# rpng/open_vins

Hardware: AMD Instinct MI355X
Metric: MSCKF features/sec per EKF update (30-clone state) (higher is better)
Workload: dtype f64; 1 GPU; BASELINE.json configs[2]: 2-camera radtan rig, 30-clone window, 2000 MSCKF features/update, N=248, D=208, online cam extrinsic+intrinsic calib + IMU intrinsics in the state, FEJ; features_total=2000, features_this_rank=2000, clones=30, cameras=2, state_dim=248, measurements_total=100362, parallelism=single GPU

## Files before the change

open_vins_amd/csrc/api_context.inc:

```
using namespace ovg;

static thread_local std::string g_err = "";
static int set_err(int code, const std::string &msg) {
  g_err = msg;
  return code;
}

#define HIPCHK(expr)                                                                                         \
  do {                                                                                                       \
    hipError_t _e = (expr);                                                                                  \
    if (_e != hipSuccess) {                                                                                  \
      return set_err(OVGPU_ERR_HIP, std::string(#expr) + " -> " + hipGetErrorString(_e) + " (" __FILE__ ":" + \
                                        std::to_string(__LINE__) + ")");                                     \
    }                                                                                                        \
  } while (0)

namespace {

template <class T>
struct PinBuf {
  T *p = nullptr;
  size_t cap = 0;
  hipError_t reserve(size_t n) {
    if (n <= cap) return hipSuccess;
// ... 186 lines not shown
  int tree_G2 = 0;
  hipStream_t stream2 = nullptr;
  hipEvent_t ev_rows = nullptr;
  bool gram_il = true;
  bool gram_blocks_only = false;
  bool fuse_chol_inputs = true;
  hipEvent_t ev_fork = nullptr, ev_join = nullptr;
  DevBuf<int32_t> leaf_flags;
  int tree_overlap = -1;
  bool tree_nodes_overlap = false, tree_nodes2_overlap = false;
  DevBuf<int32_t> tree_flags;
  DevBuf<int32_t> tree_err;
  int tree_G = 0;
  bool tree_pipelined = true;
  int compress_gram = 1;
  DevBuf<double> gram_part, gram_G, gram_rho, Yaug2, Lw;
  double prior_pivot_tol = 1e-13;
  int last_route = OVGPU_COMPRESS_GRAM;
  bool whiten = true;
  bool gram_is_whitened = false;
  bool prior_on_side = false;
  int feat_variant = 0;
  int feat_nt_max = 0;
  bool featy_ok = false;
  int featy_skip = 0;
  int featy_grid = 0;
  size_t featy_lds = 0;
  DevBuf<double> fs_tq;
  DevBuf<int32_t> fs_inst;
  DevBuf<double> featyb_ws;
  int featy_big = 0;
  bool no_feat_kernel = false;
  bool raw_enable = true;
  int raw_work_const = 12;
  bool raw_veto = false;
  bool raw_one_region = false;
  bool raw_cols_ok = false;
  bool raw_tables_ok = false;
  int raw_j0 = 0;
  int raw_ncls = 0, raw_ntc[RAW_MAXCLS + 1] = {0}, raw_ld[RAW_MAXCLS + 1] = {0}, raw_rcol[RAW_MAXCLS + 1] = {0};
  int64_t raw_base[RAW_MAXCLS + 1] = {0}, raw_rows[RAW_MAXCLS + 1] = {0};
  std::vector<uint8_t> h_cls_of_clone;
  DevBuf<uint8_t> cls_of_clone;
  DevBuf<int32_t> raw_featbase, raw_dst;
  DevBuf<double> Hraw;
  DevBuf<gram::GramRegionWG> gram_wg;
  int gram_wg_n = 0, gram_wg_tiles = 0;
  gram::GramRegionSum raw_rs;
  bool last_stack_raw = false;
  DevBuf<int32_t> feat_counter, fs_minfo, fs_meas_feat, fs_pos;
  DevBuf<int32_t> fs_slots;
  std::vector<int32_t> h_order;
  std::vector<uint16_t> h_cc;
  DevBuf<double> fs_rows, fs_V, fs_z, fs_w;
  void *comm = nullptr;
  struct LoopComm *loop = nullptr;
  int comm_rank = 0, comm_world = 1;
  DevBuf<double> comm_buf;
  DevBuf<int32_t> chol_prog;
  DevBuf<int32_t> ctrl;
  unsigned ctrl_clean = 0;
  unsigned ctrl_pre = 0;
  DevBuf<double> chol_uinv;
  DevBuf<double> chol_wide_A, chol_wide_Y;
  bool chol_wide = true;
  int64_t chol_wide_count = 0;
// ... 305 lines not shown
```

open_vins_amd/csrc/api_debug.inc:

```
int ovgpu_debug_option(ovgpu_ctx *c, const char *name, int64_t value, int64_t *old_value) {
  if (!c || !name) return set_err(OVGPU_ERR_INVALID, "null argument");
  const std::string n(name);
  if (n == "chol_follow_spin_limit") {
    if (old_value) *old_value = c->chol_spin_limit;
    if (value >= 0) c->chol_spin_limit = (int)std::min<int64_t>(value, 1 << 30);
  } else if (n == "slam_chunked_fail_chunk") {
    if (old_value) *old_value = c->chunk_fail_inject;
    c->chunk_fail_inject = value >= 0 ? (int)std::min<int64_t>(value, 1 << 20) : -1;
  } else if (n == "slam_chunked_fallbacks") {
    if (old_value) *old_value = c->chunk_fallbacks;
    if (value >= 0) c->chunk_fallbacks = value;
  } else if (n == "delayed_init_fused") {
    if (old_value) *old_value = c->init_fused_on ? 1 : 0;
    if (value >= 0) c->init_fused_on = value != 0;
  } else if (n == "delayed_init_fused_steps") {
    if (old_value) *old_value = c->init_fused_steps;
    if (value >= 0) c->init_fused_steps = value;
  } else if (n == "delayed_init_chain_steps") {
    if (old_value) *old_value = c->init_chain_steps;
    if (value >= 0) c->init_chain_steps = value;
  } else if (n == "gram_interleaved") {
    if (old_value) *old_value = c->gram_il ? 1 : 0;
    if (value >= 0) c->gram_il = value != 0;
  } else if (n == "layout_fpw") {
// ... 12 lines not shown
    if (old_value) *old_value = c->raw_enable ? 1 : 0;
    if (value >= 0) c->raw_enable = value != 0, c->raw_one_region = value == 2;
  } else if (n == "anchored_fast") {
    if (old_value) *old_value = c->anchored_fast ? 1 : 0;
    if (value >= 0) c->anchored_fast = value != 0;
  } else if (n == "gram_blocks_only") {
    if (old_value) *old_value = c->gram_blocks_only ? 1 : 0;
    if (value >= 0) c->gram_blocks_only = value != 0;
  } else if (n == "stage_timing_period") {
    if (old_value) *old_value = c->timing_period;
    if (value >= 1) c->timing_period = (int)value, c->timing_seq = 0;
  } else if (n == "fuse_chol_inputs") {
    if (old_value) *old_value = c->fuse_chol_inputs ? 1 : 0;
    if (value >= 0) c->fuse_chol_inputs = value != 0;
  } else if (n == "featy_big") {
    if (old_value) *old_value = c->featy_big;
    if (value >= 0) c->featy_big = (int)value;
  } else if (n == "upload_kernel") {
    if (old_value) *old_value = c->up_kernel;
    if (value >= 0) c->up_kernel = value != 0;
  } else if (n == "layout_every_update") {
    if (old_value) *old_value = c->layout_every_update;
    if (value >= 0) c->layout_every_update = value != 0;
  } else if (n == "tri_waves") {
    if (old_value) *old_value = c->tri_waves;
    if (value >= 0 && value <= 16) c->tri_waves = (int)value;
  } else if (n == "featy_skip") {
#ifdef OVG_FEAT_ABLATE
    if (old_value) *old_value = c->featy_skip;
    if (value >= 0) c->featy_skip = (int)value;
#else
    return set_err(OVGPU_ERR_INVALID, "featy_skip: ablation switches exist in a developer build only (-DOVG_FEAT_ABLATE)");
#endif
  } else if (n == "raw_work_const") {
    if (old_value) *old_value = c->raw_work_const;
    if (value >= 0) c->raw_work_const = (int)value;
  } else if (n == "last_stack_raw") {
    if (old_value) *old_value = c->last_stack_raw ? 1 : 0;
  } else if (n == "raw_gram_tile_rows") {
    int64_t t = 0;
    if (c->raw_tables_ok)
      for (int k = 0; k <= RAW_NEG; k++) t += c->raw_rows[k] * (int64_t)(c->raw_ntc[k] * (c->raw_ntc[k] + 1) / 2);
    if (old_value) *old_value = t;
  } else if (n == "stack_is_f32") {
    if (old_value) *old_value = c->stack_is_f32 ? 1 : 0;
  } else if (n == "last_feature_kernel") {
    if (old_value) *old_value = c->last_feat_kernel;
  } else if (n == "chol_wide") {
    if (old_value) *old_value = c->chol_wide ? 1 : 0;
    if (value >= 0) c->chol_wide = value != 0;
  } else if (n == "chol_wide_factorisations") {
    if (old_value) *old_value = c->chol_wide_count;
    if (value >= 0) c->chol_wide_count = value;
  } else if (n == "tsqr_leaves") {
    if (old_value) *old_value = c->tsqr_last_W;
  } else if (n == "tsqr_rows_per_node") {
    if (old_value) *old_value = c->tsqr_last_rpn;
  } else if (n == "tsqr_last_leaf_kernel") {
    if (old_value) *old_value = c->tsqr_last_leaf;
  } else if (n == "tsqr_last_tree") {
    if (old_value) *old_value = c->tsqr_last_tree;
  } else if (n == "tsqr_last_qh") {
    if (old_value) *old_value = c->tsqr_last_qh;
  } else if (n == "chol_timeouts") {
    if (old_value) *old_value = c->chol_timeouts;
  } else {
    return set_err(OVGPU_ERR_INVALID, "unknown debug option");
  }
  return OVGPU_OK;
}

int ovgpu_debug_cycles(ovgpu_ctx *c, int enable, long long *out512) {
  if (!c) return set_err(OVGPU_ERR_INVALID, "null ctx");
  HIPCHK(hipSetDevice(c->device));
  HIPCHK(upload_sync(c, c->stream));
  if (out512 && c->dbg_cycles.p) HIPCHK(hipMemcpy(out512, c->dbg_cycles.p, 512 * sizeof(long long), hipMemcpyDeviceToHost));
  if (enable) {
    HIPCHK(c->dbg_cycles.reserve(512));
    HIPCHK(hipMemset(c->dbg_cycles.p, 0, 512 * sizeof(long long)));
  } else if (!out512) {
    c->dbg_cycles.release();
  }
  return OVGPU_OK;
}

__global__ void k_clock_probe(long long *out, int iters) {
  const long long c0 = clock64(), w0 = wall_clock64();
  unsigned x = threadIdx.x + 1;
  for (int i = 0; i < iters; i++) x = x * 1664525u + 1013904223u;
  const long long c1 = clock64(), w1 = wall_clock64();
  if (threadIdx.x == 0) out[0] = c1 - c0, out[1] = w1 - w0, out[2] = (long long)x;
}
__global__ void __launch_bounds__(256) k_clock_probe_load(long long *out, int iters) {
  typedef double d4 __attribute__((ext_vector_type(4)));
  d4 a0 = {0, 0, 0, 0}, a1 = a0, a2 = a0, a3 = a0;
  const double x = 1.0 + 1e-9 * threadIdx.x, y = 1.0 - 1e-9 * threadIdx.x;
  const long long c0 = clock64(), w0 = wall_clock64();
  for (int i = 0; i < iters; i++) {
    a0 = __builtin_amdgcn_mfma_f64_16x16x4f64(x, y, a0, 0, 0, 0);
    a1 = __builtin_amdgcn_mfma_f64_16x16x4f64(y, x, a1, 0, 0, 0);
    a2 = __builtin_amdgcn_mfma_f64_16x16x4f64(x, x, a2, 0, 0, 0);
    a3 = __builtin_amdgcn_mfma_f64_16x16x4f64(y, y, a3, 0, 0, 0);
  }
  const long long c1 = clock64(), w1 = wall_clock64();
  if (blockIdx.x == 0 && threadIdx.x == 0) out[0] = c1 - c0, out[1] = w1 - w0;
  if (a0[0] + a1[1] + a2[2] + a3[3] == 12345.678) out[2] = 1;
}
__global__ void k_probe_empty(int *sink) {
  if (sink == nullptr && threadIdx.x == 12345) *sink = 0;
}
__global__ void k_chase_init(int32_t *buf, int n, int stride, int step) {
  const int i = blockIdx.x * blockDim.x + threadIdx.x;
  if (i < n) buf[(size_t)i * stride] = (int32_t)(((long long)i + step) % n);
}
__global__ void k_chase(const int32_t *buf, int stride, int hops, long long *out) {
  if (threadIdx.x != 0) return;
  int i = 0;
  for (int h = 0; h < 64; h++) i = __builtin_nontemporal_load(buf + (size_t)i * stride);
// ... 111 lines not shown
```

open_vins_amd/csrc/api_pipeline.inc:

```
static int enqueue_triangulate(ovgpu_ctx *c, const double *seed_pA = nullptr, const int32_t *seed_anchor = nullptr) {
  if (c->F == 0) return OVGPU_OK;
  TriParams p;
  p.seed_pA = seed_pA, p.seed_anchor = seed_anchor, p.anchor_pre = c->anchor_pre.p;
  p.F = c->F, p.C = c->C, p.K = c->K;
  p.meas_offsets = c->meas_offsets.p, p.meas_cc = c->meas_cc.p, p.uvn = c->uvn.p, p.tab_cc = c->tab_cc.p;
  p.p_FinA = c->pA.p, p.p_FinG = c->pG.p, p.anchor_meas = c->anchor.p, p.status = c->status.p;
  p.opt = c->dopt;
  const size_t lds = (size_t)c->K * c->C * 12 * sizeof(double);
  int wpb = c->tri_waves;
  if (wpb == 0) {
    wpb = 4;
    const int room = c->num_cu - 6;
    for (int w = 4; w <= 8 && room > 0; w *= 2) {
      const int blocks = (c->F + w - 1) / w;
      if (blocks <= room) {
        if (4 * blocks >= 3 * room) wpb = w;
        break;
      }
    }
  }
  hipLaunchKernelGGL(k_triangulate, dim3((c->F + wpb - 1) / wpb), dim3(64 * wpb), lds, c->stream, p);
  HIPCHK(hipGetLastError());
  return OVGPU_OK;
}
// ... 230 lines not shown
  HIPCHK(c->gram_part.reserve((size_t)G * NP * 256));
  HIPCHK(c->gram_G.reserve((size_t)LG * LG));
  if (c->stack_is_f32) {
    const int LDF = c->stack_ldf, NTM = LDF / 32, P = gram32::gram32_parts(NTM), slots = P * gram32::G32_NW * gram32::G32_MAXT;
    if (c->gram32_ntm != NTM || c->gram32_P != P) {
      std::vector<int32_t> tab((size_t)slots);
      gram32::gram32_tile_table(NTM, P, tab.data());
      HIPCHK(c->gram32_tiles.reserve((size_t)slots));
      HIPCHK(hipMemcpyAsync(c->gram32_tiles.p, tab.data(), sizeof(int32_t) * slots, hipMemcpyHostToDevice, c->stream));
      HIPCHK(upload_sync(c, c->stream));
      c->gram32_ntm = NTM, c->gram32_P = P;
    }
    const int64_t by_rows = (c->rows_total + gram32::G32_ROWS_WG - 1) / gram32::G32_ROWS_WG;
    const int64_t by_cus = std::min<int64_t>((2 * c->num_cu + P - 1) / P, (c->rows_total + 127) / 128);
    const int Gw = (int)std::max<int64_t>(1, std::max(by_rows, by_cus));
    HIPCHK(c->gram32_part.reserve((size_t)P * Gw * gram32::G32_NW * gram32::G32_MAXT * 1024));
    static bool attr32 = false;
    if (!attr32) {
      (void)hipFuncSetAttribute((const void *)gram32::k_gram_f32, hipFuncAttributeMaxDynamicSharedMemorySize, 160 * 1024);
      attr32 = true;
    }
    gram32::Gram32Params q;
    q.H = c->Hbig32.p, q.part = c->gram32_part.p, q.tiles = c->gram32_tiles.p, q.rows_total = c->rows_total, q.LDF = LDF, q.LD = LD;
    hipLaunchKernelGGL(gram32::k_gram_f32, dim3(Gw, P), dim3(gram32::G32_NTH), gram32::gram32_lds_bytes(LDF), c->stream, q);
    hipLaunchKernelGGL(gram32::k_gram_f32_reduce, dim3(slots, 4), dim3(256), 0, c->stream, (const int32_t *)c->gram32_tiles.p, Gw,
                       (const float *)c->gram32_part.p, c->gram_G.p, LG);
    HIPCHK(hipGetLastError());
    return factor ? set_err(OVGPU_ERR_CAPACITY, "the fp32 Gram variant feeds the on-device update only") : OVGPU_OK;
  }
  if (c->last_stack_raw) {
    HIPCHK(c->gram_part.reserve((size_t)std::max(c->gram_wg_tiles, 1) * 256));
    static bool attr_r = false;
    if (!attr_r) {
      (void)hipFuncSetAttribute((const void *)gram::k_gram_regions, hipFuncAttributeMaxDynamicSharedMemorySize, 160 * 1024);
      attr_r = true;
    }
    hipLaunchKernelGGL(gram::k_gram_regions, dim3(c->gram_wg_n), dim3(256), gram::gram_lds_bytes(), c->stream, (const double *)c->Hraw.p, (const gram::GramRegionWG *)c->gram_wg.p,
                       c->gram_part.p);
    hipLaunchKernelGGL(gram::k_gram_regions_reduce, dim3(NP), dim3(1024), 0, c->stream, NT, D, c->raw_rs, (const double *)c->gram_part.p, c->gram_G.p);
    HIPCHK(hipGetLastError());
    return factor ? enqueue_gram_factor(c) : OVGPU_OK;
  }
  gram::GramParams g;
  g.LD = LD, g.NT = NT, g.rows_total = c->rows_total, g.H = c->Hbig.p, g.part = c->gram_part.p;
  if (NT == gram::GR_NT + 7 && !c->gram_fp32 && !c->gram_blocks_only) {
    static bool attr_w = false;
    if (!attr_w) {
      (void)hipFuncSetAttribute((const void *)gram::k_gram_wide_top<7>, hipFuncAttributeMaxDynamicSharedMemorySize, 160 * 1024);
      (void)hipFuncSetAttribute((const void *)gram::k_gram_wide_win<7>, hipFuncAttributeMaxDynamicSharedMemorySize, 160 * 1024);
      attr_w = true;
    }
    const int Gw = G;
    hipLaunchKernelGGL(gram::k_gram_wide_top<7>, dim3(Gw), dim3(256), gram::gram_wide_top_lds_bytes(), c->stream, g);
    hipLaunchKernelGGL(gram::k_gram_wide_win<7>, dim3(Gw), dim3(256), gram::gram_lds_bytes(), c->stream, g);
    hipLaunchKernelGGL(gram::k_gram_reduce, dim3(NP), dim3(1024), 0, c->stream, NT, Gw, c->gram_part.p, c->gram_G.p);
    HIPCHK(hipGetLastError());
    return factor ? enqueue_gram_factor(c) : OVGPU_OK;
  }
  if (NT > gram::GR_NT || c->gram_fp32) {
    const int NB = (NT + gram::GB_T - 1) / gram::GB_T, pairs = NB * (NB + 1) / 2;
    HIPCHK(c->gram_part.reserve((size_t)pairs * G * gram::GB_T * gram::GB_T * 256));
    g.part = c->gram_part.p;
    static bool attr_done = false;
    if (!attr_done) {
      (void)hipFuncSetAttribute((const void *)gram::k_gram_blk<false>, hipFuncAttributeMaxDynamicSharedMemorySize, 160 * 1024);
      (void)hipFuncSetAttribute((const void *)gram::k_gram_blk<true>, hipFuncAttributeMaxDynamicSharedMemorySize, 160 * 1024);
      attr_done = true;
    }
    if (c->gram_fp32) hipLaunchKernelGGL(gram::k_gram_blk<true>, dim3(G, pairs), dim3(256), gram::gram_blk_lds_bytes() / 2, c->stream, g, NB);
    else hipLaunchKernelGGL(gram::k_gram_blk<false>, dim3(G, pairs), dim3(256), gram::gram_blk_lds_bytes(), c->stream, g, NB);
    hipLaunchKernelGGL(gram::k_gram_blk_reduce, dim3(gram::GB_T * gram::GB_T, pairs), dim3(256), 0, c->stream, NB, NT, G, c->gram_part.p, c->gram_G.p);
    HIPCHK(hipGetLastError());
// ... 777 lines not shown
```

open_vins_amd/csrc/api_state.inc:

```

const char *ovgpu_last_error(void) { return g_err.c_str(); }

void ovgpu_default_options(ovgpu_options *o) {
  if (!o) return;
  std::memset(o, 0, sizeof(*o));
  o->chi2_multipler = 5.0, o->sigma_pix = 1.0;
  o->triangulate_1d = 0, o->refine_features = 1, o->max_runs = 5;
  o->init_lamda = 1e-3, o->max_lamda = 1e10, o->min_dx = 1e-6, o->min_dcost = 1e-6, o->lam_mult = 10;
  o->min_dist = 0.10, o->max_dist = 60, o->max_baseline = 40, o->max_cond_number = 10000;
  o->do_fej = 1, o->do_calib_camera_pose = 1, o->do_calib_camera_intrinsics = 1;
  o->feat_rep_msckf = OVGPU_REP_GLOBAL_3D;
}

double ovgpu_chi2_quantile_95(int dof) { return chi2_quantile_95(dof); }
int ovgpu_abi_version(void) { return OVGPU_ABI_VERSION; }

int ovgpu_create(const ovgpu_options *opts, int device, ovgpu_ctx **out) {
  if (!opts || !out) return set_err(OVGPU_ERR_INVALID, "null argument");
  *out = nullptr;
  int ndev = 0;
  hipError_t e = hipGetDeviceCount(&ndev);
  if (e != hipSuccess || ndev <= 0)
    return set_err(OVGPU_ERR_NO_DEVICE, std::string("no HIP device (") + hipGetErrorString(e) + "): this library has no CPU fallback");
  if (device < 0 || device >= ndev) return set_err(OVGPU_ERR_INVALID, "device index out of range");
// ... 593 lines not shown
  int64_t total = 0;
  double work[RAW_MAXCLS + 1] = {0}, work_sum = 0;
  int live = 0;
  for (int k = 0; k <= RAW_NEG; k++) {
    if (k >= n && k != RAW_NEG) {
      c->raw_rows[k] = 0, c->raw_base[k] = total;
      continue;
    }
    if (run[k] >= ((int64_t)1 << RAW_CLS_SHIFT)) return OVGPU_OK;
    c->raw_rows[k] = run[k], c->raw_base[k] = total;
    total += run[k] * c->raw_ld[k];
    work[k] = (double)run[k] * (0.5 * c->raw_ntc[k] * (c->raw_ntc[k] + 1) + (double)c->raw_work_const);
    work_sum += work[k], live += run[k] > 0;
  }
  HIPCHK(c->Hraw.reserve((size_t)std::max<int64_t>(total, 1)));
  HIPCHK(c->raw_featbase.reserve(fb.size()));
  HIPCHK(c->raw_dst.reserve((size_t)M));
  HIPCHK(upload_deferred(c, c->raw_featbase.p, fb.data(), sizeof(int32_t) * fb.size()));
  const int G = std::max(c->num_cu, live);
  int wgs[RAW_MAXCLS + 1] = {0}, given = 0;
  for (int k = 0; k <= RAW_NEG; k++)
    if (c->raw_rows[k] > 0) wgs[k] = std::max(1, (int)std::floor(work[k] / work_sum * (G - live)) + 1), given += wgs[k];
  for (int k = RAW_NEG; given > G && k >= 0; k = k > 0 ? k - 1 : RAW_NEG)
    if (wgs[k] > 1) wgs[k]--, given--;
  std::vector<gram::GramRegionWG> tab;
  int tiles = 0;
  c->raw_rs.n = 0;
  for (int k = 0; k <= RAW_NEG; k++) {
    if (wgs[k] == 0) continue;
    const int64_t nchunks = (c->raw_rows[k] + gram::GR_ROWS - 1) / gram::GR_ROWS;
    const int w = (int)std::min<int64_t>(wgs[k], nchunks);
    {
      const int q = c->raw_rs.n++;
      c->raw_rs.ntc[q] = c->raw_ntc[k], c->raw_rs.rcol[q] = c->raw_rcol[k], c->raw_rs.neg[q] = k == RAW_NEG ? 1 : 0, c->raw_rs.part_tile[q] = tiles, c->raw_rs.nwg[q] = w;
    }
    for (int j = 0; j < w; j++) {
      gram::GramRegionWG r;
      r.ntc = c->raw_ntc[k], r.ld = c->raw_ld[k], r.rcol = c->raw_rcol[k], r.neg = k == RAW_NEG ? 1 : 0;
      r.h_off = c->raw_base[k], r.rows = c->raw_rows[k];
      r.chunk_begin = (int)((nchunks * j) / w), r.chunk_end = (int)((nchunks * (j + 1)) / w);
      r.part_tile = tiles;
      tiles += r.ntc * (r.ntc + 1) / 2;
      tab.push_back(r);
    }
  }
  c->gram_wg_n = (int)tab.size(), c->gram_wg_tiles = tiles;
  HIPCHK(c->gram_wg.reserve(tab.size()));
  HIPCHK(upload_deferred(c, c->gram_wg.p, tab.data(), sizeof(gram::GramRegionWG) * tab.size()));
  c->raw_tables_ok = true;
  return OVGPU_OK;
}

static int begin_feature_batch(ovgpu_ctx *c, int F, int M, const int32_t *offsets) {
  c->have_feats = false, c->tri_readable = false;
  c->raw_tables_ok = false;
  int m_max = 0;
  for (int f = 0; f < F; f++) {
    const int m = offsets[f + 1] - offsets[f];
    if (m < 0) return set_err(OVGPU_ERR_INVALID, "meas_offsets not monotone");
    m_max = std::max(m_max, m);
  }
  c->F = F, c->M = M, c->m_max = m_max;
  c->have_feat_sigma = c->have_feat_mult = false;
  c->h_feat_lm.clear(), c->h_feat_rep.clear();
  c->h_offsets.assign(offsets, offsets + (F > 0 ? F + 1 : 0));
  if (F == 0) c->h_offsets.assign(1, 0);

  const int need = std::max(500, 2 * m_max + 1);
  if ((int)c->h_chi2_table.size() < need) {
    const int old = (int)c->h_chi2_table.size();
    c->h_chi2_table.resize(need, 0.0);
    for (int i = std::max(old, 1); i < need; i++) c->h_chi2_table[i] = chi2_quantile_95(i);
  }
  c->chi2_table_len = (int)c->h_chi2_table.size();
// ... 88 lines not shown
```

open_vins_amd/csrc/k_gram.h:

```cpp
#pragma once
#include <hip/hip_runtime.h>
#include <stdint.h>
#include <type_traits>

namespace ovg {
namespace gram {

typedef double d4 __attribute__((ext_vector_type(4)));

constexpr int GR_ROWS = 32;
constexpr int GR_LS = 272;
constexpr int GR_NT = 16;
constexpr int GR_NT_BLK = 24;

struct GramParams {
  int LD, NT;
  int64_t rows_total;
  const double *H;
  double *part;
};

__host__ __device__ inline int pair_index(int NT, int ti, int tj) { return ti * NT - (ti * (ti - 1)) / 2 + (tj - ti); }
inline size_t gram_lds_bytes() { return (size_t)2 * GR_ROWS * GR_LS * sizeof(double); }

template <int W> struct WaveRows {
  static constexpr int R0 = 2 * W, R1 = 2 * W + 1, R2 = 14 - 2 * W, R3 = 15 - 2 * W;
  static constexpr int O0 = 0, O1 = O0 + GR_NT - R0, O2 = O1 + GR_NT - R1, O3 = O2 + GR_NT - R2;
};
template <int W> struct WaveRowsBal {
  static constexpr int R0 = W, R1 = 7 - W, R2 = 8 + W, R3 = 15 - W;
  static constexpr int O0 = 0, O1 = O0 + GR_NT - R0, O2 = O1 + GR_NT - R1, O3 = O2 + GR_NT - R2;
};
constexpr int GR_ACC = 34;

#define GRAM_MFMA(a, b, c) c = __builtin_amdgcn_mfma_f64_16x16x4f64(a, b, c, 0, 0, 0)

template <int W, int NTC> __device__ __forceinline__ void gram_stage(const double *cur, int lane, d4 (&acc)[GR_ACC]) {
  using WR = WaveRows<W>;
  const int g = lane >> 4, cl = lane & 15;
  constexpr int JLO = WR::R0 < NTC ? WR::R0 : NTC;
#pragma unroll 2
  for (int k0 = 0; k0 < GR_ROWS; k0 += 4) {
    const double *rowp = cur + (k0 + g) * GR_LS + cl;
    double b[GR_NT];
#pragma unroll
    for (int j = JLO; j < NTC; j++) b[j] = rowp[16 * j];
#pragma unroll
    for (int j = JLO; j < NTC; j++) {
      if (j >= WR::R0 && WR::R0 < NTC) GRAM_MFMA(b[WR::R0 < NTC ? WR::R0 : 0], b[j], acc[j >= WR::R0 ? WR::O0 + j - WR::R0 : 0]);
      if (j >= WR::R1 && WR::R1 < NTC) GRAM_MFMA(b[WR::R1 < NTC ? WR::R1 : 0], b[j], acc[j >= WR::R1 ? WR::O1 + j - WR::R1 : 0]);
      if (j >= WR::R2 && WR::R2 < NTC) GRAM_MFMA(b[WR::R2 < NTC ? WR::R2 : 0], b[j], acc[j >= WR::R2 ? WR::O2 + j - WR::R2 : 0]);
      if (j >= WR::R3 && WR::R3 < NTC) GRAM_MFMA(b[WR::R3 < NTC ? WR::R3 : 0], b[j], acc[j >= WR::R3 ? WR::O3 + j - WR::R3 : 0]);
    }
  }
}

template <int W, bool BAL = false> __device__ __forceinline__ void gram_put(double *out, int NT, int lane, const d4 (&acc)[GR_ACC]) {
  using WR = typename std::conditional<BAL, WaveRowsBal<W>, WaveRows<W>>::type;
  auto put = [&](int ti, int tj, const d4 &a) {
    if (ti < NT && tj < NT) {
      double2 *o = reinterpret_cast<double2 *>(out + (size_t)pair_index(NT, ti, tj) * 256) + lane;
      o[0] = double2{a[0], a[1]}, o[64] = double2{a[2], a[3]};
    }
  };
#pragma unroll
  for (int j = WR::R0; j < GR_NT; j++) put(WR::R0, j, acc[WR::O0 + j - WR::R0]);
#pragma unroll
  for (int j = WR::R1; j < GR_NT; j++) put(WR::R1, j, acc[WR::O1 + j - WR::R1]);
// ... 40 lines not shown
      if (cc >= LD) cc -= LD, r++;
    }
  };

  if (chunk_begin < chunk_end) {
    fetch(chunk_begin);
    stash(gram_lds);
  }
  __syncthreads();
  for (int chunk = chunk_begin; chunk < chunk_end; chunk++) {
    const double *cur = gram_lds + (size_t)((chunk - chunk_begin) & 1) * GR_ROWS * GR_LS;
    double *nxt = gram_lds + (size_t)((chunk - chunk_begin + 1) & 1) * GR_ROWS * GR_LS;
    const bool more = chunk + 1 < chunk_end;
    if (more) fetch(chunk + 1);
    switch (wave) {
    case 0: gram_stage<0, NTC>(cur, lane, acc); break;
    case 1: gram_stage<1, NTC>(cur, lane, acc); break;
    case 2: gram_stage<2, NTC>(cur, lane, acc); break;
    default: gram_stage<3, NTC>(cur, lane, acc); break;
    }
    if (more) stash(nxt);
    __syncthreads();
  }
  const int NP = NT * (NT + 1) / 2;
  double *out = p.part + (size_t)blockIdx.x * NP * 256;
  switch (wave) {
  case 0: gram_put<0>(out, NT, lane, acc); break;
  case 1: gram_put<1>(out, NT, lane, acc); break;
  case 2: gram_put<2>(out, NT, lane, acc); break;
  default: gram_put<3>(out, NT, lane, acc); break;
  }
}

template <int W, int NTC, bool BAL = false> __device__ __forceinline__ void gram_il_loop(const GramParams &p, double *gram_lds, int tid, int lane, int chunk_begin, int chunk_end,
                                                                     d4 (&acc)[GR_ACC]) {
  using WR = typename std::conditional<BAL, WaveRowsBal<W>, WaveRows<W>>::type;
  const int LD = p.LD;
  const int g = lane >> 4, cl = lane & 15;
  constexpr int JLO = WR::R0 < NTC ? WR::R0 : NTC;
  constexpr int SL = (NTC + 1) / 2;
  constexpr int NQ = 2 * NTC;
  constexpr int SCRATCH = GR_LS - 1;
  double v[NQ];
  const double *src_f = p.H;
  int left_f = 1, left_v = 1;
  const int row0 = tid / LD, col0 = tid - row0 * LD, step_r = 256 / LD, step_c = 256 - step_r * LD;
  int wr = row0, wc = col0;
  auto put = [&](double *buf, int q) {
    buf[wr < GR_ROWS ? wr * GR_LS + wc : SCRATCH] = (tid + 256 * q) < left_v ? v[q] : 0.0;
    wr += step_r, wc += step_c;
    if (wc >= LD) wc -= LD, wr++;
  };
  auto aim = [&](int chunk) {
    const int c = chunk < chunk_end ? chunk : chunk_end - 1;
    const int64_t first = (int64_t)c * GR_ROWS;
    const int64_t left64 = (p.rows_total - first) * LD;
    left_f = (int)(left64 < (int64_t)GR_ROWS * LD ? left64 : (int64_t)GR_ROWS * LD);
    src_f = p.H + first * LD;
  };
  auto fetch1 = [&](int q) {
    const int e = tid + 256 * q;
    v[q] = src_f[e < left_f ? e : left_f - 1];
  };
  if (chunk_begin < chunk_end) {
    aim(chunk_begin);
#pragma unroll
    for (int q = 0; q < NQ; q++) fetch1(q);
    left_v = left_f;
#pragma unroll
    for (int q = 0; q < NQ; q++) put(gram_lds, q);
    aim(chunk_begin + 1);
#pragma unroll
    for (int q = 0; q < NQ; q++) fetch1(q);
    left_v = left_f;
  }
  asm volatile("s_waitcnt lgkmcnt(0)\n\ts_barrier" ::: "memory");
  for (int chunk = chunk_begin; chunk < chunk_end; chunk++) {
    const double *cur = gram_lds + (size_t)((chunk - chunk_begin) & 1) * GR_ROWS * GR_LS;
    double *nxt = gram_lds + (size_t)((chunk - chunk_begin + 1) & 1) * GR_ROWS * GR_LS;
    wr = row0, wc = col0;
#pragma unroll
    for (int ks = 0; ks < 8; ks++) {
      if (ks == 4) aim(chunk + 2);
      const double *rowp = cur + (4 * ks + g) * GR_LS + cl;
      double b[GR_NT];
#pragma unroll
      for (int j = JLO; j < NTC; j++) b[j] = rowp[16 * j];
      __builtin_amdgcn_sched_barrier(0);
#pragma unroll
      for (int j = JLO; j < NTC; j++) {
        if (j >= WR::R0 && WR::R0 < NTC) GRAM_MFMA(b[WR::R0 < NTC ? WR::R0 : 0], b[j], acc[j >= WR::R0 ? WR::O0 + j - WR::R0 : 0]);
        if (j >= WR::R1 && WR::R1 < NTC) GRAM_MFMA(b[WR::R1 < NTC ? WR::R1 : 0], b[j], acc[j >= WR::R1 ? WR::O1 + j - WR::R1 : 0]);
        if (j >= WR::R2 && WR::R2 < NTC) GRAM_MFMA(b[WR::R2 < NTC ? WR::R2 : 0], b[j], acc[j >= WR::R2 ? WR::O2 + j - WR::R2 : 0]);
        if (j >= WR::R3 && WR::R3 < NTC) GRAM_MFMA(b[WR::R3 < NTC ? WR::R3 : 0], b[j], acc[j >= WR::R3 ? WR::O3 + j - WR::R3 : 0]);
        if (j - JLO < SL) {
          __builtin_amdgcn_sched_barrier(0);
          const int q = (ks & 3) * SL + (j - JLO);
          if (q < NQ) {
            if (ks < 4) put(nxt, q);
            else fetch1(q);
          }
          __builtin_amdgcn_sched_barrier(0);
        }
      }
#pragma unroll
      for (int sl = NTC - JLO; sl < SL; sl++) {
        const int q = (ks & 3) * SL + sl;
        if (q < NQ) {
          if (ks < 4) put(nxt, q);
          else fetch1(q);
        }
      }
      __builtin_amdgcn_sched_barrier(0);
    }
    left_v = left_f;
    asm volatile("s_waitcnt lgkmcnt(0)\n\ts_barrier" ::: "memory");
  }
}

template <int NTC> __global__ void __launch_bounds__(256) k_gram_il(GramParams p) {
  extern __shared__ double gram_lds[];
  const int tid = threadIdx.x, lane = tid & 63, wave = tid >> 6;
  const int NT = p.NT;
  for (int i = tid; i < 2 * GR_ROWS * GR_LS; i += 256) gram_lds[i] = 0.0;
  __syncthreads();
  const int64_t nchunks = (p.rows_total + GR_ROWS - 1) / GR_ROWS;
  const int chunk_begin = (int)((nchunks * blockIdx.x) / gridDim.x), chunk_end = (int)((nchunks * (blockIdx.x + 1)) / gridDim.x);
  d4 acc[GR_ACC];
#pragma unroll
  for (int i = 0; i < GR_ACC; i++) acc[i] = d4{0, 0, 0, 0};
  const int NP = NT * (NT + 1) / 2;
  double *out = p.part + (size_t)blockIdx.x * NP * 256;
  switch (wave) {
  case 0: gram_il_loop<0, NTC>(p, gram_lds, tid, lane, chunk_begin, chunk_end, acc), gram_put<0>(out, NT, lane, acc); break;
  case 1: gram_il_loop<1, NTC>(p, gram_lds, tid, lane, chunk_begin, chunk_end, acc), gram_put<1>(out, NT, lane, acc); break;
  case 2: gram_il_loop<2, NTC>(p, gram_lds, tid, lane, chunk_begin, chunk_end, acc), gram_put<2>(out, NT, lane, acc); break;
  default: gram_il_loop<3, NTC>(p, gram_lds, tid, lane, chunk_begin, chunk_end, acc), gram_put<3>(out, NT, lane, acc); break;
  }
}

struct GramRegionWG {
  int32_t ntc, ld, rcol, neg;
  int64_t h_off, rows;
  int32_t chunk_begin, chunk_end, part_tile, pad;
};
template <int NTC> __device__ __forceinline__ void gram_region_body(const GramParams &p, double *gram_lds, int tid, int lane, int wave, int cb, int ce) {
  d4 acc[GR_ACC];
#pragma unroll
  for (int i = 0; i < GR_ACC; i++) acc[i] = d4{0, 0, 0, 0};
  switch (wave) {
  case 0: gram_il_loop<0, NTC, true>(p, gram_lds, tid, lane, cb, ce, acc), gram_put<0, true>(p.part, NTC, lane, acc); break;
  case 1: gram_il_loop<1, NTC, true>(p, gram_lds, tid, lane, cb, ce, acc), gram_put<1, true>(p.part, NTC, lane, acc); break;
  case 2: gram_il_loop<2, NTC, true>(p, gram_lds, tid, lane, cb, ce, acc), gram_put<2, true>(p.part, NTC, lane, acc); break;
  default: gram_il_loop<3, NTC, true>(p, gram_lds, tid, lane, cb, ce, acc), gram_put<3, true>(p.part, NTC, lane, acc); break;
  }
}
__global__ void __launch_bounds__(256) k_gram_regions(const double *H, const GramRegionWG *tab, double *part) {
  extern __shared__ double gram_lds[];
  const int tid = threadIdx.x, lane = tid & 63, wave = tid >> 6;
  const GramRegionWG r = tab[blockIdx.x];
  for (int i = tid; i < 2 * GR_ROWS * GR_LS; i += 256) gram_lds[i] = 0.0;
  __syncthreads();
  GramParams p;
  p.LD = r.ld, p.NT = r.ntc, p.rows_total = r.rows, p.H = H + r.h_off, p.part = part + (size_t)r.part_tile * 256;
  switch (r.ntc) {
  case 4: gram_region_body<4>(p, gram_lds, tid, lane, wave, r.chunk_begin, r.chunk_end); break;
  case 6: gram_region_body<6>(p, gram_lds, tid, lane, wave, r.chunk_begin, r.chunk_end); break;
  case 8: gram_region_body<8>(p, gram_lds, tid, lane, wave, r.chunk_begin, r.chunk_end); break;
  case 10: gram_region_body<10>(p, gram_lds, tid, lane, wave, r.chunk_begin, r.chunk_end); break;
  case 12: gram_region_body<12>(p, gram_lds, tid, lane, wave, r.chunk_begin, r.chunk_end); break;
  case 14: gram_region_body<14>(p, gram_lds, tid, lane, wave, r.chunk_begin, r.chunk_end); break;
  default: gram_region_body<15>(p, gram_lds, tid, lane, wave, r.chunk_begin, r.chunk_end); break;
  }
}

struct GramRegionSum {
  int32_t n;
  int32_t ntc[9], rcol[9], neg[9], part_tile[9], nwg[9];
};
__global__ void __launch_bounds__(1024) k_gram_regions_reduce(int NT, int D, GramRegionSum rs, const double *part, double *G) {
  __shared__ double tot[4][256];
  const int LG = 16 * NT;
  const int idx = blockIdx.x, t = threadIdx.x & 255, grp = threadIdx.x >> 8;
  int ti = 0, rem = idx;
  while (rem >= NT - ti) rem -= NT - ti, ti++;
  const int tj = ti + rem;
  const int q = 2 * (t >> 7) + (t & 1), lane = (t >> 1) & 63;
  const int i = 16 * ti + 4 * q + (lane >> 4), j = 16 * tj + (lane & 15);
  double s = 0.0;
  for (int k = 0; k < rs.n; k++) {
    const int rc = rs.rcol[k], ntc = rs.ntc[k];
    int li = i == D ? rc : (i < rc && i < D ? i : -1), lj = j == D ? rc : (j < rc && j < D ? j : -1);
    if (li < 0 || lj < 0) continue;
    if ((li >> 4) > (lj >> 4)) {
      const int x = li;
      li = lj, lj = x;
    }
    const int lq = (li & 15) >> 2, llane = 16 * (li & 3) + (lj & 15);
    const int slot = (lq >> 1) * 128 + 2 * llane + (lq & 1);
    const int NP = ntc * (ntc + 1) / 2;
    const double *src = part + ((size_t)rs.part_tile[k] + pair_index(ntc, li >> 4, lj >> 4)) * 256 + slot;
    const int nw = rs.nwg[k], w_lo = (nw * grp) / 4, w_hi = (nw * (grp + 1)) / 4;
    double s0 = 0, s1 = 0, s2 = 0, s3 = 0;
    int w = w_lo;
    for (; w + 16 <= w_hi; w += 16) {
      double a[16];
#pragma unroll
      for (int u = 0; u < 16; u++) a[u] = src[(size_t)(w + u) * NP * 256];
#pragma unroll
      for (int u = 0; u < 16; u += 4) s0 += a[u], s1 += a[u + 1], s2 += a[u + 2], s3 += a[u + 3];
    }
    for (; w + 4 <= w_hi; w += 4) {
      double a[4];
#pragma unroll
      for (int u = 0; u < 4; u++) a[u] = src[(size_t)(w + u) * NP * 256];
      s0 += a[0], s1 += a[1], s2 += a[2], s3 += a[3];
    }
    for (; w < w_hi; w++) s0 += src[(size_t)w * NP * 256];
    const double sk = (s0 + s1) + (s2 + s3);
    s += rs.neg[k] ? -sk : sk;
  }
  tot[grp][t] = s;
  __syncthreads();
  if (grp != 0) return;
  const double v = (tot[0][t] + tot[1][t]) + (tot[2][t] + tot[3][t]);
  G[(size_t)i * LG + j] = v;
  if (ti != tj) G[(size_t)j * LG + i] = v;
}

constexpr int GW_ROWS = 16;
constexpr int GW_LS = 376;
template <int WS> struct WideCols {
  static constexpr int NT = GR_NT + WS;
  static constexpr int col_tiles(int j) { return j + 1 < WS ? j + 1 : WS; }
  static constexpr int tiles_upto(int j) {
    int t = 0;
    for (int q = 0; q < j; q++) t += col_tiles(q);
    return t;
  }
  static constexpr int total = tiles_upto(NT);
  static constexpr int cut(int w) {
    if (w <= 0) return 0;
    if (w >= 4) return NT;
    int j = 0;
    while (j < NT && 4 * tiles_upto(j) < w * total) j++;
    return j;
  }
  static constexpr int share(int w) { return tiles_upto(cut(w + 1)) - tiles_upto(cut(w)); }
  static constexpr int acc_max() {
    int m = 0;
    for (int w = 0; w < 4; w++) m = share(w) > m ? share(w) : m;
    return m;
  }
};
inline size_t gram_wide_top_lds_bytes() { return (size_t)2 * GW_ROWS * GW_LS * sizeof(double); }

template <int WS, int W, int ACC> __device__ __forceinline__ void gram_stage_top(const double *cur, int lane, d4 (&acc)[ACC]) {
  using WC = WideCols<WS>;
  constexpr int J0 = WC::cut(W), J1 = WC::cut(W + 1);
  const int g = lane >> 4, cl = lane & 15;
// ... 493 lines not shown
```

Baseline: 2.847 million features/s.

## Prefetch next Gram row slice in registers and restructure partial-sum reduction

The region Gram kernel gains a templated mode that loads the next k-step's B operands from LDS into a second register bank while the current step's MFMAs issue, so LDS read latency overlaps MFMA work. LDS zero-fill now clears only the padding columns beyond each region's row stride, not the whole buffer. The reduce kernel is rewritten to walk the flat workgroup table with precomputed per-region offsets in shared memory, spread over a 2D grid with 16 groups and 16-way unrolled loads. Negation is folded into a region tag. The trade-off is more register pressure from the double-buffered operands and extra table reads in the reduce.

```diff
diff --git a/open_vins_amd/csrc/api_context.inc b/open_vins_amd/csrc/api_context.inc
--- a/open_vins_amd/csrc/api_context.inc
+++ b/open_vins_amd/csrc/api_context.inc
@@ -242,6 +242,7 @@
   int featy_big = 0;
   bool no_feat_kernel = false;
   bool raw_enable = true;
+  bool gram_read_ahead = true;
   int raw_work_const = 12;
   bool raw_veto = false;
   bool raw_one_region = false;
diff --git a/open_vins_amd/csrc/api_debug.inc b/open_vins_amd/csrc/api_debug.inc
--- a/open_vins_amd/csrc/api_debug.inc
+++ b/open_vins_amd/csrc/api_debug.inc
@@ -68,6 +68,9 @@
 #else
     return set_err(OVGPU_ERR_INVALID, "featy_skip: ablation switches exist in a developer build only (-DOVG_FEAT_ABLATE)");
 #endif
+  } else if (n == "gram_read_ahead") {
+    if (old_value) *old_value = c->gram_read_ahead ? 1 : 0;
+    if (value >= 0) c->gram_read_ahead = value != 0;
   } else if (n == "raw_work_const") {
     if (old_value) *old_value = c->raw_work_const;
     if (value >= 0) c->raw_work_const = (int)value;
@@ -120,6 +123,17 @@
   return OVGPU_OK;
 }
 
+#ifdef OVG_GRAM_PROF
+extern "C" int ovgpu_debug_gram_phases(ovgpu_ctx *c, long long *out, int workgroups, int *launched) {
+  if (!c || !out || !launched || workgroups < 0 || workgroups > 1024) return set_err(OVGPU_ERR_INVALID, "bad argument");
+  *launched = c->gram_wg_n;
+  HIPCHK(hipSetDevice(c->device));
+  HIPCHK(upload_sync(c, c->stream));
+  HIPCHK(hipMemcpyFromSymbol(out, HIP_SYMBOL(gram::gram_prof_buf), sizeof(long long) * 32 * workgroups));
+  return OVGPU_OK;
+}
+#endif
+
 __global__ void k_clock_probe(long long *out, int iters) {
   const long long c0 = clock64(), w0 = wall_clock64();
   unsigned x = threadIdx.x + 1;
diff --git a/open_vins_amd/csrc/api_pipeline.inc b/open_vins_amd/csrc/api_pipeline.inc
--- a/open_vins_amd/csrc/api_pipeline.inc
+++ b/open_vins_amd/csrc/api_pipeline.inc
@@ -286,12 +286,14 @@
     HIPCHK(c->gram_part.reserve((size_t)std::max(c->gram_wg_tiles, 1) * 256));
     static bool attr_r = false;
     if (!attr_r) {
-      (void)hipFuncSetAttribute((const void *)gram::k_gram_regions, hipFuncAttributeMaxDynamicSharedMemorySize, 160 * 1024);
+      (void)hipFuncSetAttribute((const void *)gram::k_gram_regions<true>, hipFuncAttributeMaxDynamicSharedMemorySize, 160 * 1024);
+      (void)hipFuncSetAttribute((const void *)gram::k_gram_regions<false>, hipFuncAttributeMaxDynamicSharedMemorySize, 160 * 1024);
       attr_r = true;
     }
-    hipLaunchKernelGGL(gram::k_gram_regions, dim3(c->gram_wg_n), dim3(256), gram::gram_lds_bytes(), c->stream, (const double *)c->Hraw.p, (const gram::GramRegionWG *)c->gram_wg.p,
-                       c->gram_part.p);
-    hipLaunchKernelGGL(gram::k_gram_regions_reduce, dim3(NP), dim3(1024), 0, c->stream, NT, D, c->raw_rs, (const double *)c->gram_part.p, c->gram_G.p);
+    hipLaunchKernelGGL(c->gram_read_ahead ? gram::k_gram_regions<true> : gram::k_gram_regions<false>, dim3(c->gram_wg_n), dim3(256), gram::gram_lds_bytes(), c->stream,
+                       (const double *)c->Hraw.p, (const gram::GramRegionWG *)c->gram_wg.p, c->gram_part.p);
+    hipLaunchKernelGGL(gram::k_gram_regions_reduce, dim3(NP, 256 / gram::RR_E), dim3(gram::RR_E * gram::RR_G), 0, c->stream, NT, D, c->raw_rs,
+                       (const gram::GramRegionWG *)c->gram_wg.p, c->gram_wg_n, (const double *)c->gram_part.p, c->gram_G.p);
     HIPCHK(hipGetLastError());
     return factor ? enqueue_gram_factor(c) : OVGPU_OK;
   }
diff --git a/open_vins_amd/csrc/api_state.inc b/open_vins_amd/csrc/api_state.inc
--- a/open_vins_amd/csrc/api_state.inc
+++ b/open_vins_amd/csrc/api_state.inc
@@ -649,14 +649,15 @@
     const int w = (int)std::min<int64_t>(wgs[k], nchunks);
     {
       const int q = c->raw_rs.n++;
-      c->raw_rs.ntc[q] = c->raw_ntc[k], c->raw_rs.rcol[q] = c->raw_rcol[k], c->raw_rs.neg[q] = k == RAW_NEG ? 1 : 0, c->raw_rs.part_tile[q] = tiles, c->raw_rs.nwg[q] = w;
+      c->raw_rs.ntc[q] = c->raw_ntc[k], c->raw_rs.rcol[q] = c->raw_rcol[k];
     }
     for (int j = 0; j < w; j++) {
       gram::GramRegionWG r;
-      r.ntc = c->raw_ntc[k], r.ld = c->raw_ld[k], r.rcol = c->raw_rcol[k], r.neg = k == RAW_NEG ? 1 : 0;
+      r.ntc = c->raw_ntc[k], r.ld = c->raw_ld[k], r.rcol = c->raw_rcol[k], r.pad = 0;
+      if (r.ld > 16 * r.ntc) return set_err(OVGPU_ERR_INVALID, "raw_stack_layout: a region's row stride exceeds its tile columns");
       r.h_off = c->raw_base[k], r.rows = c->raw_rows[k];
       r.chunk_begin = (int)((nchunks * j) / w), r.chunk_end = (int)((nchunks * (j + 1)) / w);
-      r.part_tile = tiles;
+      r.part_tile = tiles, r.region = (c->raw_rs.n - 1) | (k == RAW_NEG ? 16 : 0);
       tiles += r.ntc * (r.ntc + 1) / 2;
       tab.push_back(r);
     }
diff --git a/open_vins_amd/csrc/k_gram.h b/open_vins_amd/csrc/k_gram.h
--- a/open_vins_amd/csrc/k_gram.h
+++ b/open_vins_amd/csrc/k_gram.h
@@ -34,6 +34,14 @@
 constexpr int GR_ACC = 34;
 
 #define GRAM_MFMA(a, b, c) c = __builtin_amdgcn_mfma_f64_16x16x4f64(a, b, c, 0, 0, 0)
+
+#ifdef OVG_GRAM_PROF
+__device__ long long gram_prof_buf[1024 * 4 * 8];
+#define GRAM_T(x)                          \
+  __builtin_amdgcn_sched_barrier(0);       \
+  const long long x = clock64();           \
+  __builtin_amdgcn_sched_barrier(0);
+#endif
 
 template <int W, int NTC> __device__ __forceinline__ void gram_stage(const double *cur, int lane, d4 (&acc)[GR_ACC]) {
   using WR = WaveRows<W>;
@@ -140,7 +148,7 @@
   }
 }
 
-template <int W, int NTC, bool BAL = false> __device__ __forceinline__ void gram_il_loop(const GramParams &p, double *gram_lds, int tid, int lane, int chunk_begin, int chunk_end,
+template <int W, int NTC, bool BAL = false, bool PF = false> __device__ __forceinline__ void gram_il_loop(const GramParams &p, double *gram_lds, int tid, int lane, int chunk_begin, int chunk_end,
                                                                      d4 (&acc)[GR_ACC]) {
   using WR = typename std::conditional<BAL, WaveRowsBal<W>, WaveRows<W>>::type;
   const int LD = p.LD;
@@ -170,6 +178,10 @@
     const int e = tid + 256 * q;
     v[q] = src_f[e < left_f ? e : left_f - 1];
   };
+#ifdef OVG_GRAM_PROF
+  long long prof_wait = 0, prof_bar = 0;
+  GRAM_T(prof_t0)
+#endif
   if (chunk_begin < chunk_end) {
     aim(chunk_begin);
 #pragma unroll
@@ -183,6 +195,10 @@
     left_v = left_f;
   }
   asm volatile("s_waitcnt lgkmcnt(0)\n\ts_barrier" ::: "memory");
+#ifdef OVG_GRAM_PROF
+  GRAM_T(prof_t1)
+#endif
+  double bb[2][GR_NT];
   for (int chunk = chunk_begin; chunk < chunk_end; chunk++) {
     const double *cur = gram_lds + (size_t)((chunk - chunk_begin) & 1) * GR_ROWS * GR_LS;
     double *nxt = gram_lds + (size_t)((chunk - chunk_begin + 1) & 1) * GR_ROWS * GR_LS;
@@ -191,25 +207,39 @@
     for (int ks = 0; ks < 8; ks++) {
       if (ks == 4) aim(chunk + 2);
       const double *rowp = cur + (4 * ks + g) * GR_LS + cl;
-      double b[GR_NT];
-#pragma unroll
-      for (int j = JLO; j < NTC; j++) b[j] = rowp[16 * j];
-      __builtin_amdgcn_sched_barrier(0);
+      double(&b)[GR_NT] = bb[ks & 1], (&bn)[GR_NT] = bb[(ks + 1) & 1];
+      const bool ahead = PF && ks < 7;
+      if (!PF || ks == 0) {
+#pragma unroll
+        for (int j = JLO; j < NTC; j++) b[j] = rowp[16 * j];
+        __builtin_amdgcn_sched_barrier(0);
+#ifdef OVG_GRAM_PROF
+        if constexpr (JLO < NTC) {
+          constexpr int first_back = 0xC07F | ((JLO < NTC ? NTC - JLO - 1 : 0) << 8);
+          GRAM_T(w0)
+          __builtin_amdgcn_s_waitcnt(first_back);
+          GRAM_T(w1)
+          prof_wait += w1 - w0;
+        }
+#endif
+      }
 #pragma unroll
       for (int j = JLO; j < NTC; j++) {
         if (j >= WR::R0 && WR::R0 < NTC) GRAM_MFMA(b[WR::R0 < NTC ? WR::R0 : 0], b[j], acc[j >= WR::R0 ? WR::O0 + j - WR::R0 : 0]);
         if (j >= WR::R1 && WR::R1 < NTC) GRAM_MFMA(b[WR::R1 < NTC ? WR::R1 : 0], b[j], acc[j >= WR::R1 ? WR::O1 + j - WR::R1 : 0]);
         if (j >= WR::R2 && WR::R2 < NTC) GRAM_MFMA(b[WR::R2 < NTC ? WR::R2 : 0], b[j], acc[j >= WR::R2 ? WR::O2 + j - WR::R2 : 0]);
         if (j >= WR::R3 && WR::R3 < NTC) GRAM_MFMA(b[WR::R3 < NTC ? WR::R3 : 0], b[j], acc[j >= WR::R3 ? WR::O3 + j - WR::R3 : 0]);
-        if (j - JLO < SL) {
-          __builtin_amdgcn_sched_barrier(0);
+        const bool slot = j - JLO < SL;
+        if (ahead || slot) __builtin_amdgcn_sched_barrier(0);
+        if (ahead) bn[j] = rowp[4 * GR_LS + 16 * j];
+        if (slot) {
           const int q = (ks & 3) * SL + (j - JLO);
           if (q < NQ) {
             if (ks < 4) put(nxt, q);
             else fetch1(q);
           }
-          __builtin_amdgcn_sched_barrier(0);
         }
+        if (ahead || slot) __builtin_amdgcn_sched_barrier(0);
       }
 #pragma unroll
       for (int sl = NTC - JLO; sl < SL; sl++) {
@@ -222,8 +252,22 @@
       __builtin_amdgcn_sched_barrier(0);
     }
     left_v = left_f;
+#ifdef OVG_GRAM_PROF
+    GRAM_T(b0)
+#endif
     asm volatile("s_waitcnt lgkmcnt(0)\n\ts_barrier" ::: "memory");
-  }
+#ifdef OVG_GRAM_PROF
+    GRAM_T(b1)
+    prof_bar += b1 - b0;
+#endif
+  }
+#ifdef OVG_GRAM_PROF
+  GRAM_T(prof_t2)
+  if (BAL && lane == 0) {
+    long long *o = gram_prof_buf + ((size_t)(blockIdx.x & 1023) * 4 + W) * 8;
+    o[3] = prof_t1 - prof_t0, o[4] = prof_t2 - prof_t1, o[5] = prof_wait, o[6] = prof_bar;
+  }
+#endif
 }
 
 template <int NTC> __global__ void __launch_bounds__(256) k_gram_il(GramParams p) {
@@ -248,92 +292,123 @@
 }
 
 struct GramRegionWG {
-  int32_t ntc, ld, rcol, neg;
+  int32_t ntc, ld, rcol, pad;
   int64_t h_off, rows;
-  int32_t chunk_begin, chunk_end, part_tile, pad;
+  int32_t chunk_begin, chunk_end, part_tile, region;
 };
-template <int NTC> __device__ __forceinline__ void gram_region_body(const GramParams &p, double *gram_lds, int tid, int lane, int wave, int cb, int ce) {
+template <int NTC, bool PF> __device__ __forceinline__ void gram_region_body(const GramParams &p, double *gram_lds, int tid, int lane, int wave, int cb, int ce) {
   d4 acc[GR_ACC];
 #pragma unroll
   for (int i = 0; i < GR_ACC; i++) acc[i] = d4{0, 0, 0, 0};
   switch (wave) {
-  case 0: gram_il_loop<0, NTC, true>(p, gram_lds, tid, lane, cb, ce, acc), gram_put<0, true>(p.part, NTC, lane, acc); break;
-  case 1: gram_il_loop<1, NTC, true>(p, gram_lds, tid, lane, cb, ce, acc), gram_put<1, true>(p.part, NTC, lane, acc); break;
-  case 2: gram_il_loop<2, NTC, true>(p, gram_lds, tid, lane, cb, ce, acc), gram_put<2, true>(p.part, NTC, lane, acc); break;
-  default: gram_il_loop<3, NTC, true>(p, gram_lds, tid, lane, cb, ce, acc), gram_put<3, true>(p.part, NTC, lane, acc); break;
-  }
-}
-__global__ void __launch_bounds__(256) k_gram_regions(const double *H, const GramRegionWG *tab, double *part) {
+  case 0: gram_il_loop<0, NTC, true, PF>(p, gram_lds, tid, lane, cb, ce, acc), gram_put<0, true>(p.part, NTC, lane, acc); break;
+  case 1: gram_il_loop<1, NTC, true, PF>(p, gram_lds, tid, lane, cb, ce, acc), gram_put<1, true>(p.part, NTC, lane, acc); break;
+  case 2: gram_il_loop<2, NTC, true, PF>(p, gram_lds, tid, lane, cb, ce, acc), gram_put<2, true>(p.part, NTC, lane, acc); break;
+  default: gram_il_loop<3, NTC, true, PF>(p, gram_lds, tid, lane, cb, ce, acc), gram_put<3, true>(p.part, NTC, lane, acc); break;
+  }
+}
+template <bool PF> __global__ void __launch_bounds__(256) k_gram_regions(const double *H, const GramRegionWG *tab, double *part) {
   extern __shared__ double gram_lds[];
   const int tid = threadIdx.x, lane = tid & 63, wave = tid >> 6;
   const GramRegionWG r = tab[blockIdx.x];
-  for (int i = tid; i < 2 * GR_ROWS * GR_LS; i += 256) gram_lds[i] = 0.0;
+#ifdef OVG_GRAM_PROF
+  const long long prof_w0 = wall_clock64();
+  GRAM_T(prof_c0)
+#endif
+  for (int i = tid, w = 16 * r.ntc - r.ld; i < 2 * GR_ROWS * w; i += 256) gram_lds[(i / w) * GR_LS + r.ld + i % w] = 0.0;
   __syncthreads();
+#ifdef OVG_GRAM_PROF
+  GRAM_T(prof_c1)
+#endif
   GramParams p;
   p.LD = r.ld, p.NT = r.ntc, p.rows_total = r.rows, p.H = H + r.h_off, p.part = part + (size_t)r.part_tile * 256;
   switch (r.ntc) {
-  case 4: gram_region_body<4>(p, gram_lds, tid, lane, wave, r.chunk_begin, r.chunk_end); break;
-  case 6: gram_region_body<6>(p, gram_lds, tid, lane, wave, r.chunk_begin, r.chunk_end); break;
-  case 8: gram_region_body<8>(p, gram_lds, tid, lane, wave, r.chunk_begin, r.chunk_end); break;
-  case 10: gram_region_body<10>(p, gram_lds, tid, lane, wave, r.chunk_begin, r.chunk_end); break;
-  case 12: gram_region_body<12>(p, gram_lds, tid, lane, wave, r.chunk_begin, r.chunk_end); break;
-  case 14: gram_region_body<14>(p, gram_lds, tid, lane, wave, r.chunk_begin, r.chunk_end); break;
-  default: gram_region_body<15>(p, gram_lds, tid, lane, wave, r.chunk_begin, r.chunk_end); break;
-  }
+  case 4: gram_region_body<4, PF>(p, gram_lds, tid, lane, wave, r.chunk_begin, r.chunk_end); break;
+  case 6: gram_region_body<6, PF>(p, gram_lds, tid, lane, wave, r.chunk_begin, r.chunk_end); break;
+  case 8: gram_region_body<8, PF>(p, gram_lds, tid, lane, wave, r.chunk_begin, r.chunk_end); break;
+  case 10: gram_region_body<10, PF>(p, gram_lds, tid, lane, wave, r.chunk_begin, r.chunk_end); break;
+  case 12: gram_region_body<12, PF>(p, gram_lds, tid, lane, wave, r.chunk_begin, r.chunk_end); break;
+  case 14: gram_region_body<14, PF>(p, gram_lds, tid, lane, wave, r.chunk_begin, r.chunk_end); break;
+  default: gram_region_body<15, PF>(p, gram_lds, tid, lane, wave, r.chunk_begin, r.chunk_end); break;
+  }
+#ifdef OVG_GRAM_PROF
+  __builtin_amdgcn_s_waitcnt(0x0070);
+  GRAM_T(prof_c2)
+  if (lane == 0) {
+    long long *o = gram_prof_buf + ((size_t)(blockIdx.x & 1023) * 4 + wave) * 8;
+    o[0] = prof_w0, o[1] = wall_clock64(), o[2] = prof_c1 - prof_c0, o[7] = (prof_c2 - prof_c1) - o[3] - o[4];
+  }
+#endif
 }
 
 struct GramRegionSum {
   int32_t n;
-  int32_t ntc[9], rcol[9], neg[9], part_tile[9], nwg[9];
+  int32_t ntc[9], rcol[9];
 };
-__global__ void __launch_bounds__(1024) k_gram_regions_reduce(int NT, int D, GramRegionSum rs, const double *part, double *G) {
-  __shared__ double tot[4][256];
+constexpr int RR_E = 64, RR_G = 16, RR_U = 16;
+__global__ void __launch_bounds__(RR_E *RR_G) k_gram_regions_reduce(int NT, int D, GramRegionSum rs, const GramRegionWG *__restrict__ tab, int total, const double *__restrict__ part,
+                                                                        double *__restrict__ G) {
+  __shared__ int eoff[9][RR_E];
+  __shared__ double tot[RR_G][RR_E];
   const int LG = 16 * NT;
-  const int idx = blockIdx.x, t = threadIdx.x & 255, grp = threadIdx.x >> 8;
+  const int idx = blockIdx.x, e = threadIdx.x & (RR_E - 1), t = RR_E * blockIdx.y + e;
+  const int grp = __builtin_amdgcn_readfirstlane(threadIdx.x / RR_E);
   int ti = 0, rem = idx;
   while (rem >= NT - ti) rem -= NT - ti, ti++;
   const int tj = ti + rem;
   const int q = 2 * (t >> 7) + (t & 1), lane = (t >> 1) & 63;
   const int i = 16 * ti + 4 * q + (lane >> 4), j = 16 * tj + (lane & 15);
+  if (grp < rs.n) {
+    const int rc = rs.rcol[grp], ntc = rs.ntc[grp];
+    int li = i == D ? rc : (i < rc && i < D ? i : -1), lj = j == D ? rc : (j < rc && j < D ? j : -1);
+    int off = -1;
+    if (li >= 0 && lj >= 0) {
+      if ((li >> 4) > (lj >> 4)) {
+        const int x = li;
+        li = lj, lj = x;
+      }
+      const int lq = (li & 15) >> 2, llane = 16 * (li & 3) + (lj & 15);
+      off = pair_index(ntc, li >> 4, lj >> 4) * 256 + (lq >> 1) * 128 + 2 * llane + (lq & 1);
+    }
+    eoff[grp][e] = off;
+  }
+  __syncthreads();
   double s = 0.0;
-  for (int k = 0; k < rs.n; k++) {
-    const int rc = rs.rcol[k], ntc = rs.ntc[k];
-    int li = i == D ? rc : (i < rc && i < D ? i : -1), lj = j == D ? rc : (j < rc && j < D ? j : -1);
-    if (li < 0 || lj < 0) continue;
-    if ((li >> 4) > (lj >> 4)) {
-      const int x = li;
-      li = lj, lj = x;
-    }
-    const int lq = (li & 15) >> 2, llane = 16 * (li & 3) + (lj & 15);
-    const int slot = (lq >> 1) * 128 + 2 * llane + (lq & 1);
-    const int NP = ntc * (ntc + 1) / 2;
-    const double *src = part + ((size_t)rs.part_tile[k] + pair_index(ntc, li >> 4, lj >> 4)) * 256 + slot;
-    const int nw = rs.nwg[k], w_lo = (nw * grp) / 4, w_hi = (nw * (grp + 1)) / 4;
-    double s0 = 0, s1 = 0, s2 = 0, s3 = 0;
-    int w = w_lo;
-    for (; w + 16 <= w_hi; w += 16) {
-      double a[16];
-#pragma unroll
-      for (int u = 0; u < 16; u++) a[u] = src[(size_t)(w + u) * NP * 256];
-#pragma unroll
-      for (int u = 0; u < 16; u += 4) s0 += a[u], s1 += a[u + 1], s2 += a[u + 2], s3 += a[u + 3];
-    }
-    for (; w + 4 <= w_hi; w += 4) {
-      double a[4];
-#pragma unroll
-      for (int u = 0; u < 4; u++) a[u] = src[(size_t)(w + u) * NP * 256];
-      s0 += a[0], s1 += a[1], s2 += a[2], s3 += a[3];
-    }
-    for (; w < w_hi; w++) s0 += src[(size_t)w * NP * 256];
-    const double sk = (s0 + s1) + (s2 + s3);
-    s += rs.neg[k] ? -sk : sk;
-  }
-  tot[grp][t] = s;
+  for (int base = 0; base < total; base += RR_G * RR_U) {
+    int ptile[RR_U], reg[RR_U];
+#pragma unroll
+    for (int u = 0; u < RR_U; u++) {
+      const int f = base + grp + RR_G * u, fc = f < total ? f : total - 1;
+      ptile[u] = tab[fc].part_tile, reg[u] = f < total ? tab[fc].region : -1;
+    }
+    double a[RR_U];
+    bool ok[RR_U];
+#pragma unroll
+    for (int u = 0; u < RR_U; u++) {
+      const int off = eoff[reg[u] >= 0 ? reg[u] & 15 : 0][e];
+      ok[u] = reg[u] >= 0 && off >= 0;
+      a[u] = part[(size_t)ptile[u] * 256 + (off >= 0 ? off : 0)];
+    }
+#pragma unroll
+    for (int u = 0; u < RR_U; u++) a[u] = ok[u] ? ((reg[u] & 16) ? -a[u] : a[u]) : 0.0;
+#pragma unroll
+    for (int w = 1; w < RR_U; w *= 2)
+#pragma unroll
+      for (int u = 0; u < RR_U; u += 2 * w) a[u] += a[u + w];
+    s += a[0];
+  }
+  tot[grp][e] = s;
   __syncthreads();
   if (grp != 0) return;
-  const double v = (tot[0][t] + tot[1][t]) + (tot[2][t] + tot[3][t]);
-  G[(size_t)i * LG + j] = v;
-  if (ti != tj) G[(size_t)j * LG + i] = v;
+  double v[RR_G];
+#pragma unroll
+  for (int g = 0; g < RR_G; g++) v[g] = tot[g][e];
+#pragma unroll
+  for (int w = 1; w < RR_G; w *= 2)
+#pragma unroll
+    for (int g = 0; g < RR_G; g += 2 * w) v[g] += v[g + w];
+  G[(size_t)i * LG + j] = v[0];
+  if (ti != tj) G[(size_t)j * LG + i] = v[0];
 }
 
 constexpr int GW_ROWS = 16;
```

Result: faster. 2.895 million features/s, median of 6 (+1.7%).
